# MPEGGroup/mpeg-pcc-tmc2

Measured on AMD Instinct MI355X. Metric: encoder patch+image-gen frames/sec, longdress_vox10 32-frame GOF, higher is better.
Workload: dtype int32/f64

## Files before the change

### mpeg-pcc-tmc2_amd/csrc/orient_contract.hip

```cpp
#include "internal.h"
#include "union_find.h"

namespace tmc2 {
namespace {

using Uf = UnionFind<true>;

__device__ __forceinline__ uint32_t ballot16( bool pred, int lane ) {
  return uint32_t( __ballot( pred ) >> ( lane & 48 ) ) & 0xFFFFu;
}

__device__ __forceinline__ double edgeDotOf( const double* __restrict__ normals, uint32_t u, uint32_t v ) {
  const double* a = normals + 3 * size_t( u );
  const double* b = normals + 3 * size_t( v );
  return a[0] * b[0] + a[1] * b[1] + a[2] * b[2];
}

struct GroupWalk {
  uint32_t g, end, step;
  __device__ __forceinline__ GroupWalk( uint32_t groups, bool chunked ) {
    if ( !chunked ) {
      g = blockIdx.x, end = groups, step = gridDim.x;
      return;
    }
    const XcdPlace at = xcdPlace();
    g    = uint32_t( ( uint64_t( groups ) * at.xcd ) >> 3 ) + at.slot;
    end  = uint32_t( ( uint64_t( groups ) * ( at.xcd + 1u ) ) >> 3 );
    step = at.perXcd;
  }
};

template <int K>
__global__ __launch_bounds__( 256 ) void initWordsKernel( const uint32_t* __restrict__ knn, const double* __restrict__ normals,
                                                           const uint16_t* __restrict__ mutual, const uint32_t* __restrict__ perm,
                                                           bool chunked, double tau, uint32_t n, uint16_t* __restrict__ mask,
                                                           uint16_t* __restrict__ strongAll, uint16_t* __restrict__ negAll,
                                                           uint32_t* __restrict__ word, uint32_t* __restrict__ count ) {
  static_assert( K == 16, "16 lanes per point" );
  const int j = threadIdx.x & 15, lane = threadIdx.x & 63;
  if ( blockIdx.x == 0 && threadIdx.x == 0 ) count[n] = 0;
  for ( GroupWalk w( ( n + 15 ) / 16, chunked ); w.g < w.end; w.g += w.step ) {
  const uint32_t at = w.g * 16 + ( threadIdx.x >> 4 );
  if ( at >= n ) continue;
  const uint32_t i  = perm ? perm[at] : at;
  const uint32_t vj = knn[size_t( i ) * K + j];
  const double   dj = edgeDotOf( normals, i, vj );
  const bool     strong = fabs( dj ) >= tau && dj != 0.0;
  const bool     cand   = ( ( mutual[i] >> j ) & 1u ) && strong;
  {
    const uint32_t bits = ballot16( cand, lane ), sb = ballot16( strong, lane ), nb = ballot16( dj < 0.0, lane );
    if ( j == 0 ) mask[i] = uint16_t( bits ), strongAll[i] = uint16_t( sb ), negAll[i] = uint16_t( nb );
  }
  const uint32_t v    = cand ? vj : i;
  uint32_t       prio = cand ? ufPriority( v ) : 0xFFFFFFFFu;
  uint32_t       best = v, parity = cand && dj < 0.0 ? 1u : 0u;
  uint32_t       slot = uint32_t( j );
#pragma unroll
  for ( int off = 8; off > 0; off >>= 1 ) {
    const uint32_t op = __shfl_xor( prio, off, 64 ), ob = __shfl_xor( best, off, 64 ), oq = __shfl_xor( parity, off, 64 ),
                   os = __shfl_xor( slot, off, 64 );
    if ( op < prio || ( op == prio && os < slot ) ) prio = op, best = ob, parity = oq, slot = os;
  }
  if ( j == 0 ) {
    count[i] = 0;
    if ( prio >= ufPriority( i ) ) best = i;
    word[i] = Uf::link( best, best == i ? 0u : parity );
  }
  }
}

template <int K>
__global__ __launch_bounds__( 256 ) void parityUnionKernel( const uint32_t* __restrict__ knn, const uint16_t* __restrict__ negAll,
                                                             const uint16_t* __restrict__ mask, const uint32_t* __restrict__ perm,
                                                             bool chunked, uint32_t n, uint32_t* __restrict__ word, int precheck,
                                                             bool agent ) {
  const uint32_t u = pointOfLane( perm, chunked, n );
  if ( u >= n ) return;
  uint32_t       m = mask[u];
  const uint32_t neg = negAll[u];
  while ( m ) {
    const int j = __ffs( int( m ) ) - 1;
    m &= m - 1;
    const uint32_t v = knn[size_t( u ) * K + j];
    if ( v > u ) continue;
    if ( precheck && Uf::sameSetStale( word, u, v, agent ) ) continue;
    Uf::unite( word, u, v, ( neg >> j ) & 1u, agent );
  }
}

template <int K>
__global__ __launch_bounds__( 256 ) void parityCheckKernel( const uint32_t* __restrict__ knn, const uint16_t* __restrict__ mask,
                                                             uint32_t n, uint32_t* word, uint32_t* __restrict__ bad ) {
  const uint32_t u = blockIdx.x * blockDim.x + threadIdx.x;
  if ( u >= n ) return;
  const uint32_t ru = Uf::rootCoherent( word, u, n );
  if ( ru == kUfBroken ) {
    atomicAdd( &bad[0], 1u );
    return;
  }
  uint32_t m = mask[u];
  while ( m ) {
    const int j = __ffs( int( m ) ) - 1;
    m &= m - 1;
    const uint32_t v = knn[size_t( u ) * K + j];
    if ( v > u ) continue;
    if ( Uf::rootCoherent( word, v, n ) != ru ) atomicAdd( &bad[1], 1u );
  }
}

__global__ __launch_bounds__( 256 ) void flattenKernel( uint32_t n, const uint32_t* __restrict__ perm, bool chunked,
                                                         uint32_t* __restrict__ word, uint32_t* __restrict__ root,
                                                         uint8_t* __restrict__ parity, uint32_t* __restrict__ minIdx, bool agent ) {
  const uint32_t u = pointOfLane( perm, chunked, n );
  if ( u >= n ) return;
  const UfRoot   found = Uf::find( word, u, agent );
  const uint32_t r     = found.root;
  root[u]              = r;
  parity[u]            = uint8_t( found.parity );
  if ( minIdx && u < loadStaleOk( &minIdx[r] ) ) atomicMin( &minIdx[r], u );
}

struct PairTable {
  unsigned long long *key, *bestW;
  uint32_t*           strongFirst;
  uint32_t            mask;
};
constexpr int kPairProbes = 128;

__device__ __forceinline__ uint32_t pairHash( uint32_t c, uint32_t c2 ) {
  unsigned long long h = ( (unsigned long long)c << 32 | c2 ) * 0x9E3779B97F4A7C15ull;
  return uint32_t( h >> 29 );
}
__device__ __forceinline__ uint32_t pairSlot( const PairTable& t, uint32_t c, uint32_t c2, bool insert ) {
  const unsigned long long key = ( (unsigned long long)( c + 1u ) << 32 ) | c2;
  uint32_t                 s   = pairHash( c, c2 ) & t.mask;
  for ( int probe = 0; probe < kPairProbes; ++probe ) {
    unsigned long long k = __hip_atomic_load( &t.key[s], __ATOMIC_RELAXED, __HIP_MEMORY_SCOPE_AGENT );
    if ( k == 0 && insert ) {
      const unsigned long long prev = atomicCAS( &t.key[s], 0ull, key );
      k                             = prev == 0 ? key : prev;
    }
    if ( k == key ) return s;
    if ( k == 0 ) return 0xFFFFFFFFu;
    s = ( s + 1 ) & t.mask;
  }
  return 0xFFFFFFFFu;
}

__global__ __launch_bounds__( 256 ) void clusterFlagKernel( const uint32_t* __restrict__ root, const uint32_t* __restrict__ minIdx, uint32_t n,
                                                             uint32_t* __restrict__ flag ) {
  const uint32_t u = blockIdx.x * blockDim.x + threadIdx.x;
  if ( u < n ) flag[u] = minIdx[root[u]] == u ? 1u : 0u;
}
template <int K>
__global__ __launch_bounds__( 256 ) void pairInsertKernel( const uint32_t* __restrict__ knn, const double* __restrict__ normals,
                                                            const uint16_t* __restrict__ strongAll, const uint16_t* __restrict__ negAll,
                                                            const uint32_t* __restrict__ perm, bool chunked, const uint32_t* __restrict__ root,
                                                            const uint32_t* __restrict__ minIdx, const uint32_t* __restrict__ rank,
                                                            const uint8_t* __restrict__ parity, uint32_t n, PairTable t,
                                                            uint32_t* __restrict__ cid, uint16_t* __restrict__ crossMask,
                                                            uint32_t* __restrict__ flags  ) {
  static_assert( K == 16, "16 lanes per point" );
  const int j = threadIdx.x & 15, lane = threadIdx.x & 63;
  for ( GroupWalk w( ( n + 15 ) / 16, chunked ); w.g < w.end; w.g += w.step ) {
  const uint32_t at = w.g * 16 + ( threadIdx.x >> 4 );
  const bool     in = at < n;
  const uint32_t u  = in ? ( perm ? perm[at] : at ) : 0u;
  bool           isCross = false, wrong = false, full = false;
  if ( in ) {
    const uint32_t cu = rank[minIdx[root[u]]], v = knn[size_t( u ) * K + j], cv = rank[minIdx[root[v]]];
    const bool     strong = ( strongAll[u] >> j ) & 1u;
    const uint32_t neg    = ( negAll[u] >> j ) & 1u;
    if ( j == 0 ) cid[u] = cu;
    isCross = cv != cu;
    if ( !isCross && strong ) wrong = ( uint32_t( parity[u] ) ^ parity[v] ) != neg;
    if ( isCross ) {
      const uint32_t s = pairSlot( t, cu, cv, true );
      if ( s == 0xFFFFFFFFu )
        full = true;
      else if ( !strong ) {
        const unsigned long long wgt = (unsigned long long)__double_as_longlong( fabs( edgeDotOf( normals, u, v ) ) );
        if ( wgt > __hip_atomic_load( &t.bestW[s], __ATOMIC_RELAXED, __HIP_MEMORY_SCOPE_AGENT ) ) atomicMax( &t.bestW[s], wgt );
      } else {
        uint32_t* first = &t.strongFirst[2 * size_t( s ) + ( neg ^ ( uint32_t( parity[u] ) ^ parity[v] ) )];
        const uint32_t id = u * 16u + uint32_t( j );
        if ( id < __hip_atomic_load( first, __ATOMIC_RELAXED, __HIP_MEMORY_SCOPE_AGENT ) ) atomicMin( first, id );
      }
    }
  }
  const uint32_t cross = ballot16( isCross, lane );
  if ( __ballot( wrong ) && lane == 0 ) flags[0] = 1u;
  if ( __ballot( full ) && lane == 0 ) flags[2] = 1u;
  if ( in && j == 0 ) crossMask[u] = uint16_t( cross );
  }
}
constexpr uint32_t kFoldSlots = 512, kFoldEmpty = 0xFFFFFFFFu;
__device__ __forceinline__ uint32_t foldAdd( uint32_t* key, uint32_t* val, uint32_t cu, uint32_t add, uint32_t& old ) {
  uint32_t slot = ( cu * 2654435761u ) >> 23;
  for ( ;; ) {
    const uint32_t k = atomicCAS( &key[slot], kFoldEmpty, cu );
    if ( k == kFoldEmpty || k == cu ) break;
    slot = ( slot + 1u ) & ( kFoldSlots - 1u );
  }
  old = atomicAdd( &val[slot], add );
  return slot;
}

template <int K>
__global__ __launch_bounds__( 256 ) void pairSelectKernel( const uint32_t* __restrict__ knn, const double* __restrict__ normals,
                                                            const uint16_t* __restrict__ strongAll, const uint16_t* __restrict__ negAll,
                                                            const uint32_t* __restrict__ perm, const uint16_t* __restrict__ crossMask,
                                                            const uint32_t* __restrict__ cid, const uint8_t* __restrict__ parity,
                                                            uint32_t n, PairTable t, int dedupe, uint16_t* __restrict__ keepMask,
                                                            uint32_t* __restrict__ count ) {
  static_assert( K == 16, "16 lanes per point" );
  __shared__ uint32_t fKey[kFoldSlots], fVal[kFoldSlots];
  const int j = threadIdx.x & 15, lane = threadIdx.x & 63, p = lane >> 4;
  for ( uint32_t s = threadIdx.x; s < kFoldSlots; s += blockDim.x ) fKey[s] = kFoldEmpty, fVal[s] = 0;
  __syncthreads();
  for ( uint32_t wgBase = blockIdx.x * 256u; wgBase < n; wgBase += gridDim.x * 256u ) {
  const uint32_t mineAt = wgBase + threadIdx.x;
  const uint32_t mineU  = mineAt < n ? ( perm ? perm[mineAt] : mineAt ) : 0u;
  const uint32_t mineCm = mineAt < n ? crossMask[mineU] : 0u;
  if ( mineAt < n && !mineCm ) keepMask[mineU] = 0;
  unsigned long long todo = __ballot( mineCm != 0u );
  while ( todo ) {
    const int k = ( __ffsll( (long long)todo ) - 1 ) >> 2;
    todo &= ~( 0xFull << ( 4 * k ) );
    const uint32_t u  = __shfl( mineU, 4 * k + p, 64 );
    const uint32_t cm = __shfl( mineCm, 4 * k + p, 64 );
    const bool     in = cm != 0u;
    bool           keep = false;
    uint32_t       cu = 0xFFFFFFFFu;
    if ( in ) {
      cu   = cid[u];
      keep = ( cm >> j ) & 1u;
      if ( keep && dedupe ) {
        const uint32_t v = knn[size_t( u ) * K + j];
        const uint32_t sl = pairSlot( t, cu, cid[v], false );
        if ( sl == 0xFFFFFFFFu ) {
          keep = true;
        } else if ( ( strongAll[u] >> j ) & 1u ) {
          keep = t.strongFirst[2 * size_t( sl ) + ( ( ( negAll[u] >> j ) & 1u ) ^ ( uint32_t( parity[u] ) ^ parity[v] ) )] == u * 16u + uint32_t( j );
        } else {
          keep = (unsigned long long)__double_as_longlong( fabs( edgeDotOf( normals, u, v ) ) ) == t.bestW[sl];
        }
      }
    }
    const uint32_t kept = ballot16( keep, lane );
    if ( in && j == 0 ) {
      keepMask[u] = uint16_t( kept );
      uint32_t old;
      if ( kept ) (void)foldAdd( fKey, fVal, cu, uint32_t( __popc( kept ) ), old );
    }
  }
  __syncthreads();
  for ( uint32_t s = threadIdx.x; s < kFoldSlots; s += blockDim.x ) {
    const uint32_t c = fKey[s], v = fVal[s];
    if ( c != kFoldEmpty ) {
      if ( v ) atomicAdd( &count[c], v );
      fKey[s] = kFoldEmpty, fVal[s] = 0;
    }
  }
  __syncthreads();
  }
}

template <int K>
__global__ __launch_bounds__( 256 ) void scatterCompactKernel( const uint32_t* __restrict__ knn, const double* __restrict__ normals,
                                                                const uint32_t* __restrict__ perm,
                                                                const uint32_t* __restrict__ cid, const uint8_t* __restrict__ parity,
                                                                const uint32_t* __restrict__ off, const uint16_t* __restrict__ keepMask,
                                                                const uint32_t* __restrict__ root, const uint32_t* __restrict__ minIdx,
                                                                uint32_t n, const uint32_t* __restrict__ clustersPtr, uint32_t edgeCap,
                                                                uint32_t recCap, uint32_t* __restrict__ cursor,
                                                                OrientCompactEdge* __restrict__ edges, OrientClusterRec* __restrict__ rec ) {
  static_assert( K == 16, "16 lanes per point" );
  __shared__ uint32_t fKey[kFoldSlots], fVal[kFoldSlots];
  const int      j = threadIdx.x & 15, lane = threadIdx.x & 63, p = lane >> 4;
  const uint32_t clusters = *clustersPtr;
  for ( uint32_t s = threadIdx.x; s < kFoldSlots; s += blockDim.x ) fKey[s] = kFoldEmpty, fVal[s] = 0;
  __syncthreads();
  for ( uint32_t wgBase = blockIdx.x * 256u; wgBase < n; wgBase += gridDim.x * 256u ) {
  const uint32_t mineAt = wgBase + threadIdx.x;
  const uint32_t mineU  = mineAt < n ? ( perm ? perm[mineAt] : mineAt ) : 0u;
  const uint32_t mineM  = mineAt < n ? keepMask[mineU] : 0u;
  uint32_t       slot = 0, within = 0;
  if ( mineAt < n ) {
    const uint32_t c = ( mineM || minIdx[root[mineU]] == mineU ) ? cid[mineU] : 0u;
    if ( minIdx[root[mineU]] == mineU && c < recCap ) rec[c] = OrientClusterRec{off[c], mineU, parity[mineU]};
    if ( mineU == n - 1 && clusters < recCap ) rec[clusters] = OrientClusterRec{off[clusters], 0u, 0u};
    if ( mineM ) slot = foldAdd( fKey, fVal, c, uint32_t( __popc( mineM ) ), within );
  }
  __syncthreads();
  for ( uint32_t s = threadIdx.x; s < kFoldSlots; s += blockDim.x ) {
    const uint32_t c = fKey[s];
    if ( c != kFoldEmpty ) fVal[s] = off[c] + atomicAdd( &cursor[c], fVal[s] );
  }
  __syncthreads();
  const uint32_t minePos = mineM ? fVal[slot] + within : 0u;
  unsigned long long todo = __ballot( mineM != 0u );
  while ( todo ) {
    const int k = ( __ffsll( (long long)todo ) - 1 ) >> 2;
    todo &= ~( 0xFull << ( 4 * k ) );
    const uint32_t u    = __shfl( mineU, 4 * k + p, 64 );
    const uint32_t m    = __shfl( mineM, 4 * k + p, 64 );
    const uint32_t pos0 = __shfl( minePos, 4 * k + p, 64 );
    if ( ( m >> j ) & 1u ) {
      const uint32_t v = knn[size_t( u ) * K + j];
      const double   d = edgeDotOf( normals, u, v );
      const uint32_t pos = pos0 + __popc( m & ( ( 1u << j ) - 1u ) );
      if ( pos < edgeCap ) edges[pos] = OrientCompactEdge{u, v, cid[v], uint32_t( parity[v] ), ( ( parity[u] ^ parity[v] ) & 1 ) ? -d : d};
    }
  }
  __syncthreads();
  for ( uint32_t s = threadIdx.x; s < kFoldSlots; s += blockDim.x ) fKey[s] = kFoldEmpty, fVal[s] = 0;
  __syncthreads();
  }
}

__global__ __launch_bounds__( 256 ) void compactSignsKernel( const uint32_t* __restrict__ cid, const uint8_t* __restrict__ parity,
                                                              const int8_t* __restrict__ clusterSign, uint32_t n, int8_t* __restrict__ sign ) {
  const uint32_t u = blockIdx.x * blockDim.x + threadIdx.x;
  if ( u < n ) sign[u] = int8_t( parity[u] ? -clusterSign[cid[u]] : clusterSign[cid[u]] );
}

template <int K>
__global__ __launch_bounds__( 256 ) void seedCompactKernel( const uint32_t* __restrict__ seeds, uint32_t count,
                                                             const uint32_t* __restrict__ knn, const double* __restrict__ normals,
                                                             const uint32_t* __restrict__ cid, const uint8_t* __restrict__ parity,
                                                             uint32_t* __restrict__ who ,
                                                             double* __restrict__ out ) {
  const uint32_t t = blockIdx.x * blockDim.x + threadIdx.x;
  if ( t >= count * ( K + 2 ) ) return;
  const uint32_t s = t / ( K + 2 ), j = t % ( K + 2 );
  const uint32_t i = seeds[s];
  const uint32_t v = j == 0 ? i : ( j == 1 ? ( i ? i - 1 : 0 ) : knn[size_t( i ) * K + ( j - 2 )] );
  if ( j >= 1 ) {
    uint32_t* w = who + ( size_t( s ) * ( K + 1 ) + ( j - 1 ) ) * 3;
    w[0] = v, w[1] = cid[v], w[2] = parity[v];
  }
  for ( int c = 0; c < 3; ++c ) out[3 * size_t( t ) + c] = normals[3 * size_t( v ) + c];
}

}

int gatherSeedTables( tmc2_frame* f, const uint32_t* d_cid, const uint8_t* d_parity, const std::vector<uint32_t>& seeds,
                      std::vector<uint32_t>& who, std::vector<double>& normals ) {
  const uint32_t count = uint32_t( seeds.size() );
  who.assign( size_t( count ) * 17 * 3, 0 );
  normals.assign( size_t( count ) * 18 * 3, 0.0 );
  if ( !count ) return TMC2_OK;
  hipStream_t      s = f->ctx->stream;
  DevBuf<uint32_t> d_seeds, d_who;
  DevBuf<double>   d_out;
  TMC2_TRY( d_seeds.alloc( count ) );
  TMC2_TRY( d_who.alloc( who.size() ) );
  TMC2_TRY( d_out.alloc( normals.size() ) );
  TMC2_HIP( hipMemcpyAsync( d_seeds.p, seeds.data(), size_t( count ) * 4, hipMemcpyHostToDevice, s ) );
  hipLaunchKernelGGL( seedCompactKernel<16>, dim3( ( count * 18 + 255 ) / 256 ), dim3( 256 ), 0, s, d_seeds.p, count, f->d_knn.p,
                      f->d_normals.p, d_cid, d_parity, d_who.p, d_out.p );
  TMC2_HIP( hipMemcpyAsync( who.data(), d_who.p, who.size() * 4, hipMemcpyDeviceToHost, s ) );
  TMC2_HIP( hipMemcpyAsync( normals.data(), d_out.p, normals.size() * 8, hipMemcpyDeviceToHost, s ) );
  TMC2_HIP( hipStreamSynchronize( s ) );
  return TMC2_OK;
}

int contractOrientationDevice( tmc2_frame* f, double tau, DevBuf<uint32_t>& d_cid, DevBuf<uint8_t>& d_parity, OrientCompact& g, bool& ok ) {
  tmc2_ctx*      ctx = f->ctx;
  hipStream_t    s   = ctx->stream;
  const uint32_t n   = uint32_t( f->n );
  ok                 = false;
  if ( f->k != 16 ) return TMC2_OK;
  DevBuf<uint32_t> d_word, d_count, d_off, d_cursor, d_small, d_root, d_minIdx, d_flag, d_rank, d_strongFirst;
  DevBuf<uint16_t> d_mask, d_strongAll, d_negAll, d_crossMask, d_keepMask;
  DevBuf<unsigned long long> d_pairs;
  TMC2_TRY( d_word.alloc( n ) );
  TMC2_TRY( d_small.alloc( 8 ) );
  TMC2_TRY( d_mask.alloc( n ) );
  TMC2_TRY( d_strongAll.alloc( n ) );
  TMC2_TRY( d_negAll.alloc( n ) );
  TMC2_TRY( d_root.alloc( n ) );
  TMC2_TRY( d_minIdx.alloc( n ) );
  TMC2_TRY( d_flag.alloc( n ) );
  TMC2_TRY( d_rank.alloc( n ) );
  TMC2_TRY( d_cid.alloc( n ) );
  TMC2_TRY( d_parity.alloc( n ) );
  TMC2_TRY( d_crossMask.alloc( n ) );
  TMC2_TRY( d_keepMask.alloc( n ) );
  const auto     pairsEnv = ctxOption( f->ctx, "ORIENT_PAIRS" );
  const uint32_t pairCap  = 1u << ( pairsEnv ? std::min( 24, std::max( 4, atoi( pairsEnv->c_str() ) ) ) : 20 );
  TMC2_TRY( d_pairs.alloc( 2 * size_t( pairCap ) ) );
  TMC2_TRY( d_strongFirst.alloc( 2 * size_t( pairCap ) ) );
  if ( n >= ( 1u << 28 ) ) return TMC2_OK;
  const dim3 blk( 256 ), grdN( ( n + 255 ) / 256 );
  TMC2_TRY( fillRegions( ctx, {{d_small.p, 32, 0},
                               {d_minIdx.p, size_t( n ) * 4, 0xFF},
                               {d_pairs.p, 2 * size_t( pairCap ) * 8, 0},
                               {d_strongFirst.p, 2 * size_t( pairCap ) * 4, 0xFF}} ) );
  TMC2_TRY( ensureMutualMask( f ) );
  const dim3 grdN16( chunkedGrid( cappedBlocks( ctx, ( size_t( n ) + 15 ) / 16 ) ) ), grdN8( chunkedGrid( grdN.x ) );
  const PassOrder order        = passOrder( f, "ORIENT_ORDER" );
  const bool      chunked      = order.chunked;
  const bool      chunkedPairs = chunked && ctxOption( ctx, "ORIENT_ORDER" ).has_value();
  const uint32_t* perm         = order.perm;
  const double*   normals  = f->d_normals.p;
  TMC2_TRY( d_count.alloc( size_t( n ) + 1 ) );
  hipLaunchKernelGGL( initWordsKernel<16>, grdN16, blk, 0, s, f->d_knn.p, normals, f->d_mutual.p, perm, chunked, tau, n, d_mask.p, d_strongAll.p,
                      d_negAll.p, d_word.p, d_count.p );
  hipLaunchKernelGGL( parityUnionKernel<16>, grdN8, blk, 0, s, f->d_knn.p, d_negAll.p, d_mask.p, perm, chunked, n, d_word.p, unionPrecheck( f->ctx ), unionAgentScope( f->ctx ) );
  if ( unionCheck( f->ctx ) ) {
    hipLaunchKernelGGL( parityCheckKernel<16>, grdN, blk, 0, s, f->d_knn.p, d_mask.p, n, d_word.p, d_small.p + 4 );
    TMC2_TRY( unionCheckResult( s, d_small.p + 4, "orientNormals: union-find invariant broken" ) );
  }
  hipLaunchKernelGGL( flattenKernel, grdN8, blk, 0, s, n, perm, chunked, d_word.p, d_root.p, d_parity.p, d_minIdx.p, unionAgentScope( f->ctx ) );
  hipLaunchKernelGGL( clusterFlagKernel, grdN, blk, 0, s, d_root.p, d_minIdx.p, n, d_flag.p );
  TMC2_TRY( exclusiveScanU32( ctx, d_flag.p, d_rank.p, n, d_small.p + 3 ) );
  TMC2_TRY( d_off.alloc( size_t( n ) + 1 ) );
  TMC2_TRY( d_cursor.alloc( n ) );
  PairTable t{d_pairs.p, d_pairs.p + pairCap, d_strongFirst.p, pairCap - 1};
  hipLaunchKernelGGL( pairInsertKernel<16>, grdN16, blk, 0, s, f->d_knn.p, normals, d_strongAll.p, d_negAll.p, perm, chunkedPairs, d_root.p, d_minIdx.p,
                      d_rank.p, d_parity.p, n, t, d_cid.p, d_crossMask.p, d_small.p );
  uint32_t kSpecEdges = 384 * 1024, kSpecClusters = 64 * 1024;
  if ( const auto spec = ctxOption( f->ctx, "ORIENT_SPEC" ) ) {
    unsigned e = 0, c = 0;
    if ( sscanf( spec->c_str(), "%u,%u", &e, &c ) == 2 ) kSpecEdges = std::max( 1u, std::min( kSpecEdges, e ) ), kSpecClusters = std::max( 2u, std::min( kSpecClusters, c ) );
  }
  DevBuf<OrientCompactEdge> d_edges;
  DevBuf<OrientClusterRec>  d_rec;
  TMC2_TRY( d_edges.alloc( kSpecEdges ) );
  TMC2_TRY( d_rec.alloc( kSpecClusters ) );
  uint32_t*          h_head  = ctx->hostC.get<uint32_t>( 4 + ( size_t( n ) + 4 ) / 4 + 4 );
  OrientClusterRec*  h_rec   = ctx->hostA.get<OrientClusterRec>( kSpecClusters );
  OrientCompactEdge* h_edges = ctx->hostE.get<OrientCompactEdge>( kSpecEdges );
  if ( !h_head || !h_rec || !h_edges ) {
    setError( "orientNormals: hipHostMalloc failed" );
    return TMC2_E_HIP;
  }
  TMC2_TRY( fillRegions( ctx, {{d_count.p, ( size_t( n ) + 1 ) * 4, 0}, {d_cursor.p, size_t( n ) * 4, 0}} ) );
  hipLaunchKernelGGL( pairSelectKernel<16>, grdN16, blk, 0, s, f->d_knn.p, normals, d_strongAll.p, d_negAll.p, perm, d_crossMask.p, d_cid.p,
                      d_parity.p, n, t, 1, d_keepMask.p, d_count.p );
  volatile uint32_t* headLine = ctx->answerLine( tmc2_ctx::kAnswerOrientHead );
  TMC2_TRY( exclusiveScanU32( ctx, d_count.p, d_off.p, size_t( n ) + 1, d_small.p + 1, ScanAnswer{headLine, d_small.p, 4} ) );
  hipLaunchKernelGGL( scatterCompactKernel<16>, grdN16, blk, 0, s, f->d_knn.p, normals, perm, d_cid.p, d_parity.p, d_off.p, d_keepMask.p, d_root.p,
                      d_minIdx.p, n, d_small.p + 3, kSpecEdges, kSpecClusters, d_cursor.p, d_edges.p, d_rec.p );
  const uint32_t kFirstEdges = std::min( 192u * 1024, kSpecEdges ), kFirstClusters = std::min( 32u * 1024, kSpecClusters );
  TMC2_HIP( hipMemcpyAsync( h_rec, d_rec.p, size_t( kFirstClusters ) * sizeof( OrientClusterRec ), hipMemcpyDeviceToHost, s ) );
  TMC2_HIP( hipMemcpyAsync( h_edges, d_edges.p, size_t( kFirstEdges ) * sizeof( OrientCompactEdge ), hipMemcpyDeviceToHost, s ) );
  TMC2_HIP( hipStreamSynchronize( s ) );
  uint32_t head[4] = {headLine[1], headLine[0], headLine[3], headLine[4]};
  if ( head[0] ) return TMC2_OK;
  uint32_t E = head[1], C = head[3];
  if ( !head[2] && E <= kSpecEdges && C + 1 <= kSpecClusters ) {
    bool more = false;
    if ( C + 1 > kFirstClusters ) {
      TMC2_HIP( hipMemcpyAsync( h_rec + kFirstClusters, d_rec.p + kFirstClusters, size_t( C + 1 - kFirstClusters ) * sizeof( OrientClusterRec ),
                                hipMemcpyDeviceToHost, s ) );
      more = true;
    }
    if ( E > kFirstEdges ) {
      TMC2_HIP( hipMemcpyAsync( h_edges + kFirstEdges, d_edges.p + kFirstEdges, size_t( E - kFirstEdges ) * sizeof( OrientCompactEdge ),
                                hipMemcpyDeviceToHost, s ) );
      more = true;
    }
    if ( more ) TMC2_HIP( hipStreamSynchronize( s ) );
  } else {
    if ( head[2] ) {
      ctx->stageAddHostMs( "orient_pair_table_overflow", 0.0 );
      TMC2_TRY( fillRegions( ctx, {{d_count.p, ( size_t( n ) + 1 ) * 4, 0}, {d_cursor.p, size_t( n ) * 4, 0}} ) );
      hipLaunchKernelGGL( pairSelectKernel<16>, grdN16, blk, 0, s, f->d_knn.p, normals, d_strongAll.p, d_negAll.p, perm, d_crossMask.p, d_cid.p,
                          d_parity.p, n, t, 0, d_keepMask.p, d_count.p );
      TMC2_TRY( exclusiveScanU32( ctx, d_count.p, d_off.p, size_t( n ) + 1, d_small.p + 1 ) );
      TMC2_HIP( hipMemcpyAsync( head, d_small.p, 16, hipMemcpyDeviceToHost, s ) );
      TMC2_HIP( hipStreamSynchronize( s ) );
      E = head[1], C = head[3];
    } else {
      ctx->stageAddHostMs( "orient_exact_size_repeat", 0.0 );
      TMC2_TRY( fillRegions( ctx, {{d_cursor.p, size_t( n ) * 4, 0}} ) );
    }
    TMC2_TRY( d_edges.alloc( std::max<uint32_t>( E, 1u ) ) );
    TMC2_TRY( d_rec.alloc( size_t( C ) + 1 ) );
    hipLaunchKernelGGL( scatterCompactKernel<16>, grdN16, blk, 0, s, f->d_knn.p, normals, perm, d_cid.p, d_parity.p, d_off.p, d_keepMask.p, d_root.p,
                        d_minIdx.p, n, d_small.p + 3, std::max<uint32_t>( E, 1u ), C + 1, d_cursor.p, d_edges.p, d_rec.p );
    h_rec   = ctx->hostA.get<OrientClusterRec>( size_t( C ) + 1 );
    h_edges = ctx->hostE.get<OrientCompactEdge>( std::max<uint32_t>( E, 1u ) );
    if ( !h_rec || !h_edges ) {
      setError( "orientNormals: hipHostMalloc failed" );
      return TMC2_E_HIP;
    }
    TMC2_HIP( hipMemcpyAsync( h_rec, d_rec.p, ( size_t( C ) + 1 ) * sizeof( OrientClusterRec ), hipMemcpyDeviceToHost, s ) );
    if ( E ) TMC2_HIP( hipMemcpyAsync( h_edges, d_edges.p, size_t( E ) * sizeof( OrientCompactEdge ), hipMemcpyDeviceToHost, s ) );
    TMC2_HIP( hipStreamSynchronize( s ) );
  }
  if ( ctxOption( f->ctx, "ORIENT_SPEC" ) ) ctx->stageAddHostMs( "orient_compact_edges", double( E ) );
  g.clusters = C, g.rec = h_rec, g.edges = h_edges;
  ok         = true;
  return TMC2_OK;
}

int launchClusterSigns( tmc2_frame* f, const uint32_t* d_cid, const uint8_t* d_parity, const int8_t* d_clusterSign, int8_t* d_sign ) {
  const uint32_t n = uint32_t( f->n );
  hipLaunchKernelGGL( compactSignsKernel, dim3( ( n + 255 ) / 256 ), dim3( 256 ), 0, f->ctx->stream, d_cid, d_parity, d_clusterSign, n, d_sign );
  TMC2_HIP( hipGetLastError() );
  return TMC2_OK;
}

}
```

Baseline: 216.5.

## Precompute cluster ids and batch independent loads in orientation pair kernels

Adds a separate kernel that computes cid[u] = rank[minIdx[root[u]]] once per point. The pair-insert kernel then reads cid directly instead of chasing three dependent indirections per neighbour. pairInsert also processes two point groups per iteration, and several kernels hoist their loads ahead of the branches, using empty asm pins to force the loads to issue together and overlap memory latency. The cost is one extra kernel launch, higher register pressure, and some loads issued speculatively even for inactive lanes.

```diff
diff --git a/mpeg-pcc-tmc2_amd/csrc/orient_contract.hip b/mpeg-pcc-tmc2_amd/csrc/orient_contract.hip
--- a/mpeg-pcc-tmc2_amd/csrc/orient_contract.hip
+++ b/mpeg-pcc-tmc2_amd/csrc/orient_contract.hip
@@ -14,6 +14,14 @@
   const double* a = normals + 3 * size_t( u );
   const double* b = normals + 3 * size_t( v );
   return a[0] * b[0] + a[1] * b[1] + a[2] * b[2];
+}
+
+__device__ __forceinline__ void ocPin( uint32_t& a ) { asm volatile( "" : "+v"( a ) ); }
+__device__ __forceinline__ void ocPin( double& a ) { asm volatile( "" : "+v"( a ) ); }
+template <typename T, typename... Rest>
+__device__ __forceinline__ void ocPin( T& a, Rest&... rest ) {
+  ocPin( a );
+  ocPin( rest... );
 }
 
 struct GroupWalk {
@@ -152,38 +160,62 @@
   const uint32_t u = blockIdx.x * blockDim.x + threadIdx.x;
   if ( u < n ) flag[u] = minIdx[root[u]] == u ? 1u : 0u;
 }
+__global__ __launch_bounds__( 256 ) void clusterIdKernel( const uint32_t* __restrict__ root, const uint32_t* __restrict__ minIdx,
+                                                           const uint32_t* __restrict__ rank, uint32_t n, uint32_t* __restrict__ cid ) {
+  const uint32_t u = blockIdx.x * blockDim.x + threadIdx.x;
+  if ( u < n ) cid[u] = rank[minIdx[root[u]]];
+}
+constexpr int kInsertGroups = 2;
 template <int K>
 __global__ __launch_bounds__( 256 ) void pairInsertKernel( const uint32_t* __restrict__ knn, const double* __restrict__ normals,
                                                             const uint16_t* __restrict__ strongAll, const uint16_t* __restrict__ negAll,
-                                                            const uint32_t* __restrict__ perm, bool chunked, const uint32_t* __restrict__ root,
-                                                            const uint32_t* __restrict__ minIdx, const uint32_t* __restrict__ rank,
+                                                            const uint32_t* __restrict__ perm, bool chunked, const uint32_t* __restrict__ cid,
                                                             const uint8_t* __restrict__ parity, uint32_t n, PairTable t,
-                                                            uint32_t* __restrict__ cid, uint16_t* __restrict__ crossMask,
+                                                            uint16_t* __restrict__ crossMask,
                                                             uint32_t* __restrict__ flags  ) {
   static_assert( K == 16, "16 lanes per point" );
+  constexpr int G = kInsertGroups;
   const int j = threadIdx.x & 15, lane = threadIdx.x & 63;
-  for ( GroupWalk w( ( n + 15 ) / 16, chunked ); w.g < w.end; w.g += w.step ) {
-  const uint32_t at = w.g * 16 + ( threadIdx.x >> 4 );
-  const bool     in = at < n;
-  const uint32_t u  = in ? ( perm ? perm[at] : at ) : 0u;
-  bool           isCross = false, wrong = false, full = false;
-  if ( in ) {
-    const uint32_t cu = rank[minIdx[root[u]]], v = knn[size_t( u ) * K + j], cv = rank[minIdx[root[v]]];
-    const bool     strong = ( strongAll[u] >> j ) & 1u;
-    const uint32_t neg    = ( negAll[u] >> j ) & 1u;
-    if ( j == 0 ) cid[u] = cu;
-    isCross = cv != cu;
-    if ( !isCross && strong ) wrong = ( uint32_t( parity[u] ) ^ parity[v] ) != neg;
+  for ( GroupWalk w( ( n + 15 ) / 16, chunked ); w.g < w.end; w.g += G * w.step ) {
+  uint32_t u[G], v[G], cu[G], sAll[G], nAll[G], pu[G], cv[G], pv[G];
+  bool     in[G];
+#pragma unroll
+  for ( int r = 0; r < G; ++r ) {
+    const uint32_t g = w.g + uint32_t( r ) * w.step, at = g * 16 + ( threadIdx.x >> 4 );
+    in[r] = g < w.end && at < n;
+    u[r]  = in[r] ? ( perm ? perm[at] : at ) : 0u;
+  }
+  if ( perm ) {
+#pragma unroll
+    for ( int r = 0; r < G; ++r ) ocPin( u[r] );
+  }
+#pragma unroll
+  for ( int r = 0; r < G; ++r )
+    v[r] = knn[size_t( u[r] ) * K + j], cu[r] = cid[u[r]], sAll[r] = strongAll[u[r]], nAll[r] = negAll[u[r]], pu[r] = parity[u[r]];
+#pragma unroll
+  for ( int r = 0; r < G; ++r ) ocPin( v[r], cu[r], sAll[r], nAll[r], pu[r] );
+#pragma unroll
+  for ( int r = 0; r < G; ++r ) cv[r] = cid[v[r]], pv[r] = parity[v[r]];
+#pragma unroll
+  for ( int r = 0; r < G; ++r ) ocPin( cv[r], pv[r] );
+#pragma unroll
+  for ( int r = 0; r < G; ++r ) {
+  bool isCross = false, wrong = false, full = false;
+  if ( in[r] ) {
+    const bool     strong = ( sAll[r] >> j ) & 1u;
+    const uint32_t neg    = ( nAll[r] >> j ) & 1u;
+    isCross = cv[r] != cu[r];
+    if ( !isCross && strong ) wrong = ( pu[r] ^ pv[r] ) != neg;
     if ( isCross ) {
-      const uint32_t s = pairSlot( t, cu, cv, true );
+      const uint32_t s = pairSlot( t, cu[r], cv[r], true );
       if ( s == 0xFFFFFFFFu )
         full = true;
       else if ( !strong ) {
-        const unsigned long long wgt = (unsigned long long)__double_as_longlong( fabs( edgeDotOf( normals, u, v ) ) );
+        const unsigned long long wgt = (unsigned long long)__double_as_longlong( fabs( edgeDotOf( normals, u[r], v[r] ) ) );
         if ( wgt > __hip_atomic_load( &t.bestW[s], __ATOMIC_RELAXED, __HIP_MEMORY_SCOPE_AGENT ) ) atomicMax( &t.bestW[s], wgt );
       } else {
-        uint32_t* first = &t.strongFirst[2 * size_t( s ) + ( neg ^ ( uint32_t( parity[u] ) ^ parity[v] ) )];
-        const uint32_t id = u * 16u + uint32_t( j );
+        uint32_t* first = &t.strongFirst[2 * size_t( s ) + ( neg ^ ( pu[r] ^ pv[r] ) )];
+        const uint32_t id = u[r] * 16u + uint32_t( j );
         if ( id < __hip_atomic_load( first, __ATOMIC_RELAXED, __HIP_MEMORY_SCOPE_AGENT ) ) atomicMin( first, id );
       }
     }
@@ -191,7 +223,8 @@
   const uint32_t cross = ballot16( isCross, lane );
   if ( __ballot( wrong ) && lane == 0 ) flags[0] = 1u;
   if ( __ballot( full ) && lane == 0 ) flags[2] = 1u;
-  if ( in && j == 0 ) crossMask[u] = uint16_t( cross );
+  if ( in[r] && j == 0 ) crossMask[u[r]] = uint16_t( cross );
+  }
   }
 }
 constexpr uint32_t kFoldSlots = 512, kFoldEmpty = 0xFFFFFFFFu;
@@ -230,21 +263,19 @@
     const uint32_t u  = __shfl( mineU, 4 * k + p, 64 );
     const uint32_t cm = __shfl( mineCm, 4 * k + p, 64 );
     const bool     in = cm != 0u;
-    bool           keep = false;
-    uint32_t       cu = 0xFFFFFFFFu;
-    if ( in ) {
-      cu   = cid[u];
-      keep = ( cm >> j ) & 1u;
-      if ( keep && dedupe ) {
-        const uint32_t v = knn[size_t( u ) * K + j];
-        const uint32_t sl = pairSlot( t, cu, cid[v], false );
-        if ( sl == 0xFFFFFFFFu ) {
-          keep = true;
-        } else if ( ( strongAll[u] >> j ) & 1u ) {
-          keep = t.strongFirst[2 * size_t( sl ) + ( ( ( negAll[u] >> j ) & 1u ) ^ ( uint32_t( parity[u] ) ^ parity[v] ) )] == u * 16u + uint32_t( j );
-        } else {
-          keep = (unsigned long long)__double_as_longlong( fabs( edgeDotOf( normals, u, v ) ) ) == t.bestW[sl];
-        }
+    bool           keep = in && ( ( cm >> j ) & 1u );
+    uint32_t v = knn[size_t( u ) * K + j], cu = cid[u], sAll = strongAll[u], nAll = negAll[u], pu = parity[u];
+    ocPin( v, cu, sAll, nAll, pu );
+    if ( keep && dedupe ) {
+      uint32_t cv = cid[v], pv = parity[v];
+      ocPin( cv, pv );
+      const uint32_t sl = pairSlot( t, cu, cv, false );
+      if ( sl == 0xFFFFFFFFu ) {
+        keep = true;
+      } else if ( ( sAll >> j ) & 1u ) {
+        keep = t.strongFirst[2 * size_t( sl ) + ( ( ( nAll >> j ) & 1u ) ^ ( pu ^ pv ) )] == u * 16u + uint32_t( j );
+      } else {
+        keep = (unsigned long long)__double_as_longlong( fabs( edgeDotOf( normals, u, v ) ) ) == t.bestW[sl];
       }
     }
     const uint32_t kept = ballot16( keep, lane );
@@ -284,11 +315,12 @@
   for ( uint32_t wgBase = blockIdx.x * 256u; wgBase < n; wgBase += gridDim.x * 256u ) {
   const uint32_t mineAt = wgBase + threadIdx.x;
   const uint32_t mineU  = mineAt < n ? ( perm ? perm[mineAt] : mineAt ) : 0u;
-  const uint32_t mineM  = mineAt < n ? keepMask[mineU] : 0u;
+  uint32_t mineM = keepMask[mineU], mineR = root[mineU], c = cid[mineU], mineP = parity[mineU];
+  ocPin( mineM, mineR, c, mineP );
+  if ( mineAt >= n ) mineM = 0u;
   uint32_t       slot = 0, within = 0;
   if ( mineAt < n ) {
-    const uint32_t c = ( mineM || minIdx[root[mineU]] == mineU ) ? cid[mineU] : 0u;
-    if ( minIdx[root[mineU]] == mineU && c < recCap ) rec[c] = OrientClusterRec{off[c], mineU, parity[mineU]};
+    if ( minIdx[mineR] == mineU && c < recCap ) rec[c] = OrientClusterRec{off[c], mineU, mineP};
     if ( mineU == n - 1 && clusters < recCap ) rec[clusters] = OrientClusterRec{off[clusters], 0u, 0u};
     if ( mineM ) slot = foldAdd( fKey, fVal, c, uint32_t( __popc( mineM ) ), within );
   }
@@ -307,10 +339,17 @@
     const uint32_t m    = __shfl( mineM, 4 * k + p, 64 );
     const uint32_t pos0 = __shfl( minePos, 4 * k + p, 64 );
     if ( ( m >> j ) & 1u ) {
-      const uint32_t v = knn[size_t( u ) * K + j];
-      const double   d = edgeDotOf( normals, u, v );
+      const double* a  = normals + 3 * size_t( u );
+      uint32_t      v  = knn[size_t( u ) * K + j], pu = parity[u];
+      double        a0 = a[0], a1 = a[1], a2 = a[2];
+      ocPin( v, pu, a0, a1, a2 );
+      const double* b  = normals + 3 * size_t( v );
+      uint32_t      cv = cid[v], pv = parity[v];
+      double        b0 = b[0], b1 = b[1], b2 = b[2];
+      ocPin( cv, pv, b0, b1, b2 );
+      const double   d   = a0 * b0 + a1 * b1 + a2 * b2;
       const uint32_t pos = pos0 + __popc( m & ( ( 1u << j ) - 1u ) );
-      if ( pos < edgeCap ) edges[pos] = OrientCompactEdge{u, v, cid[v], uint32_t( parity[v] ), ( ( parity[u] ^ parity[v] ) & 1 ) ? -d : d};
+      if ( pos < edgeCap ) edges[pos] = OrientCompactEdge{u, v, cv, pv, ( ( pu ^ pv ) & 1 ) ? -d : d};
     }
   }
   __syncthreads();
@@ -419,8 +458,9 @@
   TMC2_TRY( d_off.alloc( size_t( n ) + 1 ) );
   TMC2_TRY( d_cursor.alloc( n ) );
   PairTable t{d_pairs.p, d_pairs.p + pairCap, d_strongFirst.p, pairCap - 1};
-  hipLaunchKernelGGL( pairInsertKernel<16>, grdN16, blk, 0, s, f->d_knn.p, normals, d_strongAll.p, d_negAll.p, perm, chunkedPairs, d_root.p, d_minIdx.p,
-                      d_rank.p, d_parity.p, n, t, d_cid.p, d_crossMask.p, d_small.p );
+  hipLaunchKernelGGL( clusterIdKernel, grdN, blk, 0, s, d_root.p, d_minIdx.p, d_rank.p, n, d_cid.p );
+  hipLaunchKernelGGL( pairInsertKernel<16>, grdN16, blk, 0, s, f->d_knn.p, normals, d_strongAll.p, d_negAll.p, perm, chunkedPairs, d_cid.p, d_parity.p, n,
+                      t, d_crossMask.p, d_small.p );
   uint32_t kSpecEdges = 384 * 1024, kSpecClusters = 64 * 1024;
   if ( const auto spec = ctxOption( f->ctx, "ORIENT_SPEC" ) ) {
     unsigned e = 0, c = 0;
```

Result: no change. 217.8, median of 6 (+0.6%).
